# DanecLacey/basic_iterative_solvers

Measured on AMD Instinct MI355X. Metric: CG iterations/sec + SpMV GFLOP/s (% HBM roofline), HPCG 256^3 at 1/2/4/8 GPUs, higher is better.
Workload: dtype f64

## Files before the change

### basic_iterative_solvers_amd/__init__.py

```python
import ctypes as C
import os

import numpy as np

PKG = os.path.dirname(os.path.abspath(__file__))
LIB_PATH = os.path.join(PKG, "lib", "libbis_hip.so")

PC = dict(none=0, j=1, gs=2, bgs=3, sgs=4, **{"2st": 5, "s2st": 6, "ilu0": 7, "ilu0it": 8, "fsai": 9, "mg": 10, "bj": 11})

_lib = None


class BisError(RuntimeError):
    pass


def load_library():
    global _lib
    if _lib is None:
        if not os.path.exists(LIB_PATH):
            raise BisError(
                f"{LIB_PATH} is missing: build it with "
                "`python -m basic_iterative_solvers_amd.build` (hipcc, gfx950)")
        _lib = C.CDLL(LIB_PATH)
# ... 688 lines not shown
                raise BisError("Context.bjacobi: give block_size or block_ptr")
            p = BJParams(int(block_size), None, 0, int(bool(symmetrize)))
        ctx.check(ctx.lib.bis_bj_create(ctx.h, A.h, C.byref(p), C.byref(self.h)))
        self.n_blocks, self.max_block, self.value_count = self.info()
        self.operand = Mat(ctx, C.c_void_p(ctx.lib.bis_bj_operand(self.h)))

    def info(self):
        nb, mb, vc = C.c_int64(), C.c_int(), C.c_int64()
        self.ctx.lib.bis_bj_info(self.h, C.byref(nb), C.byref(mb), C.byref(vc))
        return nb.value, mb.value, vc.value

    def blocks(self):
        vals = np.zeros(self.value_count, dtype=np.float64)
        offs = np.zeros(self.n_blocks + 1, dtype=np.int64)
        self.ctx.check(self.ctx.lib.bis_bj_blocks(self.ctx.h, self.h, vals.ctypes, offs.ctypes))
        return vals, offs

    def apply(self, out, inp):
        self.ctx.check(self.ctx.lib.bis_bj_apply(self.ctx.h, self.h, C.c_void_p(out.ptr), C.c_void_p(inp.ptr)))

    def mapply(self, out, inp, k):
        self.ctx.check(self.ctx.lib.bis_bj_mapply(self.ctx.h, self.h, C.c_void_p(out.ptr), C.c_void_p(inp.ptr), C.c_int(int(k))))

    def free(self):
        if self.h:
            self.ctx.lib.bis_bj_destroy(self.ctx.h, self.h)
            self.h = C.c_void_p()


def _handle_pc(pc, Ls):
    if isinstance(pc, MG):
        return "mg", pc.operand
    if isinstance(pc, BJ):
        return "bj", pc.operand
    return pc, Ls


class _Solver:

    _sym = None

    def _fn(self, what):
        return getattr(self.ctx.lib, f"bis_{self._sym}_{what}")

    def set_preconditioner(self, pc, Ls=None, Us=None, A_D=None, A_D_inv=None, L_D=None, U_D=None, outer=1, inner=0):
        def p(v):
            return C.c_void_p(v.ptr) if v is not None else C.c_void_p()
        pc, Ls = _handle_pc(pc, Ls)
        self._keep_pc = (Ls, Us, A_D, A_D_inv, L_D, U_D)
        self.ctx.check(self._fn("set_preconditioner")(
            self.ctx.h, self.h, C.c_int(PC[pc] if isinstance(pc, str) else pc),
            Ls.h if Ls is not None else C.c_void_p(), Us.h if Us is not None else C.c_void_p(),
            p(A_D), p(A_D_inv), p(L_D), p(U_D), C.c_int(outer), C.c_int(inner)))

    def iterate(self, n):
        self.ctx.check(self._fn("iterate")(self.ctx.h, self.h, C.c_int(int(n))))

    def free(self):
        if self.h:
            self._fn("destroy")(self.ctx.h, self.h)
            self.h = C.c_void_p()


class CG(_Solver):
    _sym = "cg"

    def __init__(self, ctx, A, b, x, A_D=None):
        self.ctx = ctx
        self.h = C.c_void_p()
        ctx.check(ctx.lib.bis_cg_create(ctx.h, A.h, C.c_void_p(A_D.ptr) if A_D else C.c_void_p(),
                                        C.c_void_p(b.ptr), C.c_void_p(x.ptr), C.byref(self.h)))

    def init(self, tol):
        r0 = C.c_double()
        self.ctx.check(self.ctx.lib.bis_cg_init(self.ctx.h, self.h, C.c_double(tol), C.byref(r0)))
        return r0.value

    def status(self, hist_cap=4096):
        iters, conv = C.c_int(), C.c_int()
        hist = np.zeros(hist_cap)
        self.ctx.check(self.ctx.lib.bis_cg_status(self.ctx.h, self.h, C.byref(iters), C.byref(conv),
                                                  hist.ctypes, C.c_int(hist_cap)))
        return iters.value, bool(conv.value), hist[:min(iters.value + 1, hist_cap)].copy()


class MCG(_Solver):

    _sym = "mcg"

    def __init__(self, ctx, A, B, X, k, A_D=None):
        self.ctx, self.k = ctx, int(k)
        self.h = C.c_void_p()
        self._keep = (A, B, X, A_D)
        ctx.check(ctx.lib.bis_mcg_create(ctx.h, A.h, C.c_void_p(A_D.ptr) if A_D else C.c_void_p(),
                                         C.c_void_p(B.ptr), C.c_void_p(X.ptr), C.c_int(self.k), C.byref(self.h)))

    def init(self, tol):
        r0 = np.zeros(self.k)
        self.ctx.check(self.ctx.lib.bis_mcg_init(self.ctx.h, self.h, C.c_double(tol), r0.ctypes))
        return r0

    def status(self, j, hist_cap=4096):
        iters, conv = C.c_int(), C.c_int()
        hist = np.zeros(hist_cap)
        self.ctx.check(self.ctx.lib.bis_mcg_status(self.ctx.h, self.h, C.c_int(int(j)), C.byref(iters), C.byref(conv),
                                                   hist.ctypes, C.c_int(hist_cap)))
        return iters.value, bool(conv.value), hist[:min(iters.value + 1, hist_cap)].copy()


class MBiCGSTAB(_Solver):

    _sym = "mbicgstab"

    def __init__(self, ctx, A, B, X, k):
        self.ctx, self.k = ctx, int(k)
        self.h = C.c_void_p()
        self._keep = (A, B, X)
        ctx.check(ctx.lib.bis_mbicgstab_create(ctx.h, A.h, C.c_void_p(B.ptr), C.c_void_p(X.ptr), C.c_int(self.k), C.byref(self.h)))

    def init(self, tol):
        r0 = np.zeros(self.k)
        self.ctx.check(self.ctx.lib.bis_mbicgstab_init(self.ctx.h, self.h, C.c_double(tol), r0.ctypes))
        return r0

    def status(self, j, hist_cap=4096):
        iters, conv = C.c_int(), C.c_int()
        hist = np.zeros(hist_cap)
        self.ctx.check(self.ctx.lib.bis_mbicgstab_status(self.ctx.h, self.h, C.c_int(int(j)), C.byref(iters), C.byref(conv),
                                                         hist.ctypes, C.c_int(hist_cap)))
        return iters.value, bool(conv.value), hist[:min(iters.value + 1, hist_cap)].copy()


class MGMRES(_Solver):

    _sym = "mgmres"

    def __init__(self, ctx, A, B, X, k, restart=10):
        self.ctx, self.k, self.restart = ctx, int(k), int(restart)
        self.h = C.c_void_p()
        self._keep = (A, B, X)
        ctx.check(ctx.lib.bis_mgmres_create(ctx.h, A.h, C.c_void_p(B.ptr), C.c_void_p(X.ptr), C.c_int(self.k),
                                            C.c_int(self.restart), C.byref(self.h)))

    def init(self, tol):
        r0 = np.zeros(self.k)
        self.ctx.check(self.ctx.lib.bis_mgmres_init(self.ctx.h, self.h, C.c_double(tol), r0.ctypes))
        return r0

    def status(self, j, hist_cap=4096):
        iters, conv, n_hist = C.c_int(), C.c_int(), C.c_int()
        hist = np.zeros(hist_cap)
        self.ctx.check(self.ctx.lib.bis_mgmres_status(self.ctx.h, self.h, C.c_int(int(j)), C.byref(iters), C.byref(conv),
                                                      C.byref(n_hist), hist.ctypes, C.c_int(hist_cap)))
        return iters.value, bool(conv.value), hist[:min(n_hist.value, hist_cap)].copy()

    def solution(self, out):
        self.ctx.check(self.ctx.lib.bis_mgmres_solution(self.ctx.h, self.h, C.c_void_p(out.ptr)))


class FGMRES(_Solver):

    _sym = "fgmres"

    def __init__(self, ctx, A, b, x, restart=10):
        self.ctx, self.restart = ctx, int(restart)
        self.h = C.c_void_p()
# ... 380 lines not shown
```

### basic_iterative_solvers_amd/csrc/bis_blas1.hip

```cpp
#include "bis_internal.hpp"

#include <algorithm>
#include <cstdlib>

namespace {

constexpr int kEwThreads = 256;

inline int ew_grid(int64_t n_items) {
    int64_t g = (n_items + kEwThreads - 1) / kEwThreads;
    if (g < 1) g = 1;
    if (g > kMaxDotBlocks) g = kMaxDotBlocks;
    return (int)g;
}
inline int ew_grid_wide(int64_t n_items) {
    int64_t g = (n_items + kEwThreads - 1) / kEwThreads;
    if (g < 1) g = 1;
    if (g > kMaxEwBlocks) g = kMaxEwBlocks;
    return (int)g;
}

typedef double ew_v2d_t __attribute__((ext_vector_type(2)));
__device__ __forceinline__ double2 ld_stream(const double2 *p) {
    const ew_v2d_t v = __builtin_nontemporal_load(reinterpret_cast<const ew_v2d_t *>(p));
// ... 127 lines not shown
    int64_t i = (int64_t)blockIdx.x * kEwThreads + threadIdx.x;
    double acc0 = 0.0, acc1 = 0.0;
    if (VEC) {
        const int64_t n2 = n >> 1;
        double2 *w2 = reinterpret_cast<double2 *>(w);
        const double2 *u2 = reinterpret_cast<const double2 *>(u);
        const double2 *v2 = reinterpret_cast<const double2 *>(v);
        for (; i < n2; i += stride) {
            double2 wv = ld_stream(w2 + i);
            const double2 uv = ld_stream(u2 + i);
            wv.x = ew_apply<OP_SUB>(wv.x, uv.x, s);
            wv.y = ew_apply<OP_SUB>(wv.y, uv.y, s);
            w2[i] = wv;
            const double2 vv = v ? ld_stream(v2 + i) : wv;
            acc0 = fma(wv.x, vv.x, acc0);
            acc1 = fma(wv.y, vv.y, acc1);
        }
        if ((n & 1) && blockIdx.x == 0 && threadIdx.x == 0) {
            const double t = ew_apply<OP_SUB>(w[n - 1], u[n - 1], s);
            w[n - 1] = t;
            acc0 = fma(t, v ? v[n - 1] : t, acc0);
        }
    } else {
        for (; i < n; i += stride) {
            const double t = ew_apply<OP_SUB>(w[i], u[i], s);
            w[i] = t;
            acc0 = fma(t, v ? v[i] : t, acc0);
        }
    }
    const double r = block_sum<kEwThreads>(acc0 + acc1, lds);
    if (threadIdx.x == 0) partials[blockIdx.x] = r;
}

__global__ __launch_bounds__(256) void reduce_finish_kernel(const double *partials,
                                                            int n_partials, size_t stride,
                                                            double *result) {
    __shared__ double lds[4];
    const double *p = partials + (size_t)blockIdx.x * stride;
    double acc = 0.0;
    for (int i = threadIdx.x; i < n_partials; i += 256) acc += p[i];
    const double s = block_sum<256>(acc, lds);
    if (threadIdx.x == 0) result[blockIdx.x] = s;
}

enum { SC_DIV, SC_RATIO_PRODUCT, SC_SQRT_INV };
__global__ void scalar_kernel(int op, double *out, double *out2, const double *a, const double *b, const double *c,
                              const double *d) {
    if (op == SC_DIV) *out = *a / *b;
    else if (op == SC_RATIO_PRODUCT) *out = (*a / *b) * (*c / *d);
    else { const double nrm = sqrt(*a); *out = nrm; *out2 = 1.0 / nrm; }
}

}

bis_status bis_reduce_finish(bis_ctx *ctx, int n_partials, int n_values, size_t stride,
                             double *result_dev) {
    hipLaunchKernelGGL(reduce_finish_kernel, dim3(n_values), dim3(256), 0, ctx->stream,
                       ctx->partials, n_partials, stride, result_dev);
    BIS_HIP_CHECK(ctx, hipGetLastError());
    return BIS_OK;
}

bis_status bis_ensure_partials(bis_ctx *ctx, size_t n) {
    if (n <= ctx->partials_cap) return BIS_OK;
    BIS_HIP_CHECK(ctx, hipStreamSynchronize(ctx->stream));
    if (ctx->partials) BIS_HIP_CHECK(ctx, hipFree(ctx->partials));
    ctx->partials = nullptr;
    ctx->partials_cap = 0;
    BIS_HIP_CHECK(ctx, hipMalloc(&ctx->partials, sizeof(double) * n));
    ctx->partials_cap = n;
    return BIS_OK;
}

bis_status bis_fault_check(bis_ctx *ctx) {
    volatile unsigned *f = ctx->fault_host;
    if (!f || *f == 0) return BIS_OK;
    *f = 0;
    ctx->err = "a triangular sweep lost a hand-off: a row waited for a result that was never published "
               "(a workgroup of the persistent grid could not become resident, or the dependency data is corrupt); "
               "the vectors written since the last blocking call are invalid";
    return BIS_ERR_SYNC;
}

#define BIS_OPTIONS_ENV(X) X(spmv_variant) X(spmv_window) X(spmv_chunk) X(spmv_chunk_fused) X(spmv_xcd_remap) X(trsv_grid) X(ilu0_wgs) X(trsv_wave_wgs) X(trsv_trial) X(trsv_one_xcd) X(trsv_host_analysis) X(ilu0_wave) X(spmv_packed) X(spmv_packed32) X(spmv_valdict) X(spmv_sellwin) X(device_share) X(spmv_sellwin_rows) X(spmv_sellwin_joint) X(spmv_sellwin_pairs) X(spmv_sellwin_masks) X(spmv_colslab) X(spmv_win8) X(spmv_win8_rows) X(spmv_win8_depth) X(spmv_win8_sets) X(spmv_win8_implicit) X(spmv_win8_tune) X(spmv_win4) X(grid_autodetect) X(tune_placement) X(force_rp64) X(trsv_tiled) X(trsv_chain) X(trsv_tile_rows) X(trsv_tile_wgs) X(trsv_tile_edge) X(trsv_tile_backoff)
#define BIS_OPTIONS_API(Y) Y(trsv_batch) Y(trsv_wave) Y(ilu0_persistent) Y(trsv_by_pos) Y(spmv_lds_pad) Y(trsv_chain_idle) Y(trsv_chain_pause) Y(trsv_chain_pairs) Y(trsv_chain_prefix) Y(trsv_tile_exp) Y(cg_nt_x) Y(spmv_sellwin_nt) Y(dist_host_plan) Y(trsv_inject_loss) Y(trsv_inject_oom) Y(trsm_form) Y(spgemm_row_cap) Y(spgemm_batch)

namespace {
std::string &opts_env_seen() { static std::string s; return s; }
std::string upper_env(const char *name) {
    std::string e = "BIS_";
    for (const char *c = name; *c; ++c) e += (char)((*c >= 'a' && *c <= 'z') ? *c - 32 : *c);
    return e;
}
}

bis_options &bis_opts() {
    static bis_options o = [] {
        bis_options v;
#define X(name) { const std::string en = upper_env(#name); if (const char *e = getenv(en.c_str())) { v.name = atoi(e); \
                  std::string &seen = opts_env_seen(); if (!seen.empty()) seen += ' '; seen += en + "=" + e; } }
        BIS_OPTIONS_ENV(X)
#undef X
        return v;
    }();
    return o;
}

extern "C" {

bis_status bis_set_option(const char *name, int value) {
    if (!name) return BIS_ERR_INVALID;
    bis_options &o = bis_opts();
#define X(opt) if (!strcmp(name, #opt)) { o.opt = value; return BIS_OK; }
    BIS_OPTIONS_ENV(X)
    BIS_OPTIONS_API(X)
#undef X
    return BIS_ERR_INVALID;
}

int bis_options_describe(char *buf, int cap) {
    const bis_options &o = bis_opts();
    std::string s = "{";
    bool first = true;
#define X(opt) if (o.opt != -1) { if (!first) s += ", "; first = false; s += std::string("\"") + #opt + "\": " + std::to_string(o.opt); }
    BIS_OPTIONS_ENV(X)
    BIS_OPTIONS_API(X)
#undef X
    if (!first) s += ", ";
    s += "\"env\": \"";
    for (char c : opts_env_seen()) if (c != '"' && c != '\\' && (unsigned char)c >= 32) s += c;
    s += "\"}";
    if (buf && cap > 0) { const int n = std::min((int)s.size(), cap - 1); memcpy(buf, s.data(), (size_t)n); buf[n] = 0; }
    return (int)s.size();
}

int bis_abi_version(void) { return 1; }

bis_status bis_ctx_create(int device, void *stream, bis_ctx **out) {
    if (!out) return BIS_ERR_INVALID;
    *out = nullptr;
    int count = 0;
    if (hipGetDeviceCount(&count) != hipSuccess || count <= 0) return BIS_ERR_NO_DEVICE;
    if (device < 0 || device >= count) return BIS_ERR_NO_DEVICE;
    if (hipSetDevice(device) != hipSuccess) return BIS_ERR_NO_DEVICE;
    hipDeviceProp_t prop;
    if (hipGetDeviceProperties(&prop, device) != hipSuccess) return BIS_ERR_NO_DEVICE;
    bis_ctx *ctx = new bis_ctx;
    ctx->device = device;
    ctx->n_cus = prop.multiProcessorCount;
    ctx->arch = prop.gcnArchName;
    ctx->hbm_bytes = (int64_t)prop.totalGlobalMem;
    if (ctx->arch.rfind("gfx950", 0) != 0) {
        fprintf(stderr, "bis_hip: device %d is %s, this library is built for gfx950 only\n",
                device, ctx->arch.c_str());
        delete ctx;
        return BIS_ERR_NO_DEVICE;
    }
    if (stream) {
        ctx->stream = (hipStream_t)stream;
    } else {
        if (hipStreamCreateWithFlags(&ctx->stream, hipStreamNonBlocking) != hipSuccess) {
            delete ctx;
            return BIS_ERR_HIP;
        }
        ctx->own_stream = true;
    }
    ctx->partials_cap = std::max((size_t)kMaxReduceBlocks * 4, (size_t)kMaxDotBlocks * 2);
// ... 327 lines not shown
```

### basic_iterative_solvers_amd/csrc/bis_cg.hip

```cpp
#include "bis_solver.hpp"

#include <algorithm>
#include <cfloat>
#include <cmath>

struct bis_dist;
bis_status bis_dist_spmv_launch(bis_ctx *ctx, bis_dist *d, double *x_ext, double *y, const double *w,
                                int *n_partials);
size_t bis_dist_partials_need(const bis_dist *d);
int64_t bis_dist_n_local(const bis_dist *d);
int64_t bis_dist_n_ext(const bis_dist *d);
bis_status bis_dist_allreduce(bis_ctx *ctx, bis_dist *d, double *buf_dev, int count);

struct bis_cg : bis_solver_core {
    bis_dist *dist = nullptr;
    const bis_mat *A = nullptr;
    const double *A_D = nullptr;
    const double *b = nullptr;
    double *x = nullptr;
    int64_t n = 0;
    double *p = nullptr, *r = nullptr, *z = nullptr, *tmp = nullptr;
    double *sc = nullptr;
    double *pap_stage = nullptr;
};

namespace {

enum { S_RZ = 0, S_PAP, S_RZ_NEW, S_RR, S_ALPHA, S_BETA, S_STOP, S_COUNT = 8 };
constexpr int kT = kSolverT;


__device__ __forceinline__ void cg_book(double rz_new, double rr, double *sc, int *flags, double *hist, int hist_cap) {
    const double rz_old = sc[S_RZ];
    sc[S_BETA] = rz_new / rz_old;
    sc[S_RZ] = rz_new;
    sc[S_RR] = rr;
    const double norm = sqrt(rr);
    const int it = flags[0] + 1;
    flags[0] = it;
    if (it < hist_cap) hist[it] = norm;
    const bool conv = fabs(norm) < sc[S_STOP];
    const bool diverged = fabs(norm) > DBL_MAX || norm != norm;
    if (conv || diverged) { flags[1] = 1; flags[2] = conv ? 1 : 0; flags[3] = it; }
}

constexpr int kPapBlocks = 256;
__global__ __launch_bounds__(256) void cg_finish_pap_kernel(const double *__restrict__ partials, int n_partials,
                                                            double *stage, double *sc, const int *flags,
                                                            unsigned *counter) {
    __shared__ double lds[4];
    __shared__ bool last;
    if (flags[1]) return;
    const int per = (n_partials + kPapBlocks - 1) / kPapBlocks;
    const int lo = blockIdx.x * per, hi = min(lo + per, n_partials);
    double acc = 0.0;
    for (int i = lo + (int)threadIdx.x; i < hi; i += 256) acc += partials[i];
    const double s = block_sum<256>(acc, lds);
    if (threadIdx.x == 0) {
        publish(stage + blockIdx.x, s);
        last = arrive_last(counter, kPapBlocks);
    }
    __syncthreads();
    if (!last) return;
    const double t = block_sum<256>(threadIdx.x < kPapBlocks ? fetch(stage + threadIdx.x) : 0.0, lds);
    if (threadIdx.x == 0) sc[S_PAP] = t;
}

typedef double cg_v2d_t __attribute__((ext_vector_type(2)));
template <bool JACOBI, bool DIST>
__global__ __launch_bounds__(kT) void cg_update_kernel(int64_t n, double *sc, int *flags,
                                                       const double *__restrict__ tmp,
                                                       const double *__restrict__ D,
                                                       double *__restrict__ r,
                                                       double *__restrict__ z,
                                                       double *partials, size_t stride, unsigned *counter,
                                                       double *hist, int hist_cap, int nt_tmp, int nt_r) {
    __shared__ double lds[kT / 64];
    __shared__ bool last;
    if (flags[1]) return;
    const double alpha = sc[S_RZ] / sc[S_PAP];
    const int64_t n2 = n >> 1, gs = (int64_t)gridDim.x * kT;
    double rz = 0.0, rr = 0.0;
    const double2 *t2 = reinterpret_cast<const double2 *>(tmp);
    const double2 *D2 = reinterpret_cast<const double2 *>(D);
    double2 *r2 = reinterpret_cast<double2 *>(r);
    double2 *z2 = reinterpret_cast<double2 *>(z);
    for (int64_t i = (int64_t)blockIdx.x * kT + threadIdx.x; i < n2; i += gs) {
        double2 tv;
        if (nt_tmp) {
            const cg_v2d_t v = __builtin_nontemporal_load(reinterpret_cast<const cg_v2d_t *>(t2 + i));
            tv = make_double2(v.x, v.y);
        } else tv = t2[i];
        double2 rv, zv;
        if (nt_r) {
            const cg_v2d_t v = __builtin_nontemporal_load(reinterpret_cast<const cg_v2d_t *>(r2 + i));
            rv = make_double2(v.x, v.y);
        } else rv = r2[i];
        rv.x = fma(-alpha, tv.x, rv.x);
        rv.y = fma(-alpha, tv.y, rv.y);
        r2[i] = rv;
        if (JACOBI) {
            const double2 dv = D2[i];
            zv.x = rv.x / (1.0 * dv.x);
            zv.y = rv.y / (1.0 * dv.y);
            z2[i] = zv;
        } else {
// ... 65 lines not shown
        } else xv = x2[i];
        xv.x = fma(alpha, pv.x, xv.x);
        xv.y = fma(alpha, pv.y, xv.y);
        pv.x = fma(beta, pv.x, zv.x);
        pv.y = fma(beta, pv.y, zv.y);
        if (NT) { cg_v2d_t v; v.x = xv.x; v.y = xv.y; __builtin_nontemporal_store(v, reinterpret_cast<cg_v2d_t *>(x2 + i)); }
        else x2[i] = xv;
        p2[i] = pv;
    }
    if ((n & 1) && blockIdx.x == 0 && threadIdx.x == 0) {
        x[n - 1] = fma(alpha, p[n - 1], x[n - 1]);
        p[n - 1] = fma(beta, p[n - 1], z[n - 1]);
    }
}

}

extern "C" {

static bis_status cg_create_common(bis_ctx *ctx, bis_dist *dist, const bis_mat *A, const double *A_D,
                                   const double *b, double *x, bis_cg **out) {
    bis_cg *cg = new bis_cg;
    cg->dist = dist;
    cg->A = A;
    cg->A_D = A_D;
    cg->b = b;
    cg->x = x;
    cg->n = dist ? bis_dist_n_local(dist) : A->n_rows;
    const int64_t n_ext = dist ? bis_dist_n_ext(dist) : cg->n;
    bis_status st = bis_vec_alloc(ctx, n_ext, &cg->p);
    if (st == BIS_OK) st = bis_vec_alloc(ctx, cg->n, &cg->r);
    if (st == BIS_OK && A_D) st = bis_vec_alloc(ctx, cg->n, &cg->z);
    if (st == BIS_OK) st = bis_vec_alloc(ctx, cg->n, &cg->tmp);
    if (st == BIS_OK) st = bis_vec_alloc(ctx, S_COUNT, &cg->sc);
    if (st == BIS_OK) st = bis_vec_alloc(ctx, kPapBlocks, &cg->pap_stage);
    if (st == BIS_OK) st = bis_solver_core_alloc(ctx, cg, 4, 1, 1, 4 + kArriveSubs);
    if (st != BIS_OK) { bis_cg_destroy(ctx, cg); return st; }
    cg->pc.tmp = cg->tmp;
    if (!A_D) cg->z = cg->r;
    *out = cg;
    return BIS_OK;
}

bis_status bis_cg_create(bis_ctx *ctx, const bis_mat *A, const double *A_D, const double *b,
                         double *x, bis_cg **out) {
    BIS_CTX_OK(ctx);
    BIS_REQUIRE(ctx, A && b && x && out, "bis_cg_create: bad arguments");
    BIS_REQUIRE(ctx, A->n_rows == A->n_cols, "bis_cg_create: square matrix required");
    return cg_create_common(ctx, nullptr, A, A_D, b, x, out);
}

bis_status bis_dist_cg_create(bis_ctx *ctx, bis_dist *d, const double *A_D, const double *b,
                              double *x, bis_cg **out) {
    BIS_CTX_OK(ctx);
    BIS_REQUIRE(ctx, d && b && x && out, "bis_dist_cg_create: bad arguments");
    return cg_create_common(ctx, d, nullptr, A_D, b, x, out);
}

bis_status bis_cg_set_preconditioner(bis_ctx *ctx, bis_cg *cg, int precond_type, const bis_mat *L_strict, const bis_mat *U_strict,
                                     const double *A_D, const double *A_D_inv, const double *L_D, const double *U_D,
                                     int outer_iters, int inner_iters) {
    BIS_CTX_OK(ctx);
    if (!cg) return bis_pc_no_handle(ctx, "bis_cg", 0, precond_type);
    return bis_pc_bind(ctx, &cg->pc, {"bis_cg", cg->n, cg->n, 0, bis_solver_live(*cg), cg->dist ? 2 : 1},
                       {precond_type, L_strict, U_strict, A_D, A_D_inv, L_D, U_D, outer_iters, inner_iters},
                       {{&cg->z, cg->n, cg->z == cg->r}});
}

bis_status bis_cg_destroy(bis_ctx *ctx, bis_cg *cg) {
    BIS_CTX_OK(ctx);
    if (!cg) return BIS_OK;
    hipStreamSynchronize(ctx->stream);
    hipFree(cg->p);
    hipFree(cg->r);
    if (cg->z != cg->r) hipFree(cg->z);
    hipFree(cg->tmp);
    hipFree(cg->sc);
    hipFree(cg->pap_stage);
    bis_solver_core_free(cg);
    delete cg;
    return BIS_OK;
}

bis_status bis_cg_init(bis_ctx *ctx, bis_cg *cg, double tol, double *r0_norm_host) {
    BIS_CTX_OK(ctx);
    BIS_REQUIRE(ctx, cg, "bis_cg_init: null handle");
    const int64_t n = cg->n;
    bis_status st;
    double rz = 0.0, rr = 0.0;
    if (cg->dist) {
        st = bis_copy_vector(ctx, cg->p, cg->x, n);
        if (st == BIS_OK) st = bis_dist_spmv_launch(ctx, cg->dist, cg->p, cg->tmp, nullptr, nullptr);
        if (st == BIS_OK) st = bis_subtract_vectors(ctx, cg->r, cg->b, cg->tmp, n, 1.0);
    } else {
        st = bis_compute_residual(ctx, cg->A, cg->x, cg->b, cg->r, cg->tmp);
    }
    if (st == BIS_OK && cg->pc.set) st = bis_pc_apply(ctx, cg->pc, n, 0, cg->z, cg->r);
    else if (st == BIS_OK && cg->A_D) st = bis_elemwise_div_vectors(ctx, cg->z, cg->r, cg->A_D, n, 1.0);
    if (st == BIS_OK) st = bis_copy_vector(ctx, cg->p, cg->z, n);
    if (cg->dist) {
        if (st == BIS_OK) st = bis_dist_dot(ctx, cg->dist, cg->r, cg->z, ctx->scalars_dev + 8, &rz);
        if (st == BIS_OK) st = bis_dist_dot(ctx, cg->dist, cg->r, cg->r, ctx->scalars_dev + 8, &rr);
    } else {
        if (st == BIS_OK) st = bis_dot(ctx, cg->r, cg->z, n, &rz);
        if (st == BIS_OK) st = bis_dot(ctx, cg->r, cg->r, n, &rr);
    }
    if (st != BIS_OK) return st;
    const double norm0 = sqrt(rr);
    double sc[S_COUNT] = {0};
    sc[S_RZ] = rz;
    sc[S_RR] = rr;
    sc[S_STOP] = tol * norm0;
    int flags[4] = {0, 0, 0, 0};
    BIS_HIP_CHECK(ctx, hipMemcpyAsync(cg->sc, sc, sizeof sc, hipMemcpyHostToDevice, ctx->stream));
    BIS_HIP_CHECK(ctx, hipMemcpyAsync(cg->flags, flags, sizeof flags, hipMemcpyHostToDevice, ctx->stream));
    BIS_HIP_CHECK(ctx, hipMemcpyAsync(cg->hist, &norm0, sizeof(double), hipMemcpyHostToDevice, ctx->stream));
    BIS_HIP_CHECK(ctx, hipStreamSynchronize(ctx->stream));
    cg->enqueued = 0;
    cg->initialised = true;
    if (r0_norm_host) *r0_norm_host = norm0;
    return BIS_OK;
}

static bis_status cg_enqueue_iteration(bis_ctx *ctx, bis_cg *cg, int g, int it) {
    const int64_t n = cg->n;
    int n_part = 0;
    bis_status st;
    if (cg->dist) st = bis_dist_spmv_launch(ctx, cg->dist, cg->p, cg->tmp, cg->p, &n_part);
    else st = bis_spmv_launch(ctx, cg->A, cg->p, cg->tmp, cg->p, &n_part);
    if (st != BIS_OK) return st;
    hipLaunchKernelGGL(cg_finish_pap_kernel, dim3(kPapBlocks), dim3(256), 0, ctx->stream,
                       ctx->partials, n_part, cg->pap_stage, cg->sc, cg->flags, cg->counters);
    if (cg->dist) {
        st = bis_dist_allreduce(ctx, cg->dist, cg->sc + S_PAP, 1);
        if (st != BIS_OK) return st;
    }
#define BIS_CG_UPDATE(J, D)                                                                                  \
    hipLaunchKernelGGL((cg_update_kernel<J, D>), dim3(g), dim3(kT), 0, ctx->stream, n, cg->sc, cg->flags,    \
                       cg->tmp, cg->A_D, cg->r, cg->z, ctx->partials, (size_t)kMaxReduceBlocks,              \
                       cg->counters + 1, cg->hist, cg->hist_cap, bis_opts().cg_nt_x != 0 && bis_opts().cg_nt_x != 2, bis_opts().cg_nt_x == 3)
    if (cg->pc.set) BIS_CG_UPDATE(false, true);
    else if (cg->dist) { if (cg->A_D) BIS_CG_UPDATE(true, true); else BIS_CG_UPDATE(false, true); }
    else { if (cg->A_D) BIS_CG_UPDATE(true, false); else BIS_CG_UPDATE(false, false); }
#undef BIS_CG_UPDATE
    if (cg->pc.set) {
        st = bis_pc_apply(ctx, cg->pc, n, 0, cg->z, cg->r);
        if (st == BIS_OK) st = bis_dot_dev(ctx, cg->r, cg->z, n, cg->sc + S_RZ_NEW);
        if (st != BIS_OK) return st;
        if (!cg->dist)
            hipLaunchKernelGGL(cg_book_kernel, dim3(1), dim3(64), 0, ctx->stream, cg->sc, cg->flags, cg->hist, cg->hist_cap);
    }
    if (cg->dist) {
        st = bis_dist_allreduce(ctx, cg->dist, cg->sc + S_RZ_NEW, 2);
        if (st != BIS_OK) return st;
        hipLaunchKernelGGL(cg_book_kernel, dim3(1), dim3(64), 0, ctx->stream, cg->sc, cg->flags, cg->hist, cg->hist_cap);
    }
    if (bis_opts().cg_nt_x == 3) hipLaunchKernelGGL((cg_p_update_kernel<true, true>), dim3(g), dim3(kT), 0, ctx->stream, n, cg->sc, cg->flags, it, cg->z, cg->x, cg->p);
    else if (bis_opts().cg_nt_x != 0) hipLaunchKernelGGL(cg_p_update_kernel<true>, dim3(g), dim3(kT), 0, ctx->stream, n, cg->sc, cg->flags, it, cg->z, cg->x, cg->p);
    else hipLaunchKernelGGL(cg_p_update_kernel<false>, dim3(g), dim3(kT), 0, ctx->stream, n, cg->sc, cg->flags, it, cg->z, cg->x, cg->p);
    return BIS_OK;
}

bis_status bis_cg_iterate(bis_ctx *ctx, bis_cg *cg, int n_iters) {
    BIS_CTX_OK(ctx);
    BIS_REQUIRE(ctx, cg && n_iters >= 0 && cg->enqueued + n_iters < kMaxIters,
                "bis_cg_iterate: bad arguments");
    const int64_t n = cg->n;
    if (n == 0) return BIS_OK;
    const int g = bis_pair_grid(n, kMaxReduceBlocks);
    const size_t need = std::max((size_t)2 * kMaxReduceBlocks,
                                 cg->dist ? bis_dist_partials_need(cg->dist) : bis_spmv_partials_bound(cg->A));
    bis_status st = bis_ensure_partials(ctx, need);
    if (st != BIS_OK) return st;
    bis_stop_guard stop_guard(ctx, cg->flags);
    for (int done = 0; done < n_iters; ++done) {
        st = cg_enqueue_iteration(ctx, cg, g, cg->enqueued + done + 1);
        if (st != BIS_OK) { cg->enqueued += done; return st; }
    }
    BIS_HIP_CHECK(ctx, hipGetLastError());
    cg->enqueued += n_iters;
    return BIS_OK;
}

bis_status bis_cg_status(bis_ctx *ctx, bis_cg *cg, int *iters, int *converged, double *hist_host,
                         int hist_cap) {
    BIS_CTX_OK(ctx);
    BIS_REQUIRE(ctx, cg, "bis_cg_status: null handle");
    int flags[4] = {0, 0, 0, 0};
    if (bis_status st = bis_solver_read_flags(ctx, *cg, 0, 4, flags)) return st;
    if (iters) *iters = flags[0];
    if (converged) *converged = flags[2];
    if (hist_host && hist_cap > 0) return bis_solver_copy_hist(ctx, *cg, 0, std::min(flags[0] + 1, hist_cap), hist_host);
    return BIS_OK;
}

}
```

### basic_iterative_solvers_amd/csrc/bis_internal.hpp

```cpp
#pragma once

#include <hip/hip_runtime.h>

#include <cstdint>
#include <cstdio>
#include <cstring>
#include <map>
#include <string>
#include <vector>

#include "bis_hip.h"

struct bis_trsv_plan;
struct bis_trsv_tiled;
struct bis_trsv_chain;
struct bis_trsm_plan;
struct bis_trsv_side {
    bis_trsv_plan *level = nullptr;
    bis_trsv_tiled *tiled = nullptr;
    bis_trsv_chain *chain = nullptr;
    bis_trsm_plan *multi = nullptr;
    bool tiled_tried = false, chain_tried = false;
    const char *kernel = "";
    const char *kernel_m = "";
};

struct bis_named_kernel {
    int type = 0;
    const bis_mat *A = nullptr;
    double *B = nullptr, *C = nullptr;
    int64_t size_B = 0, size_C = 0;
    const double *D = nullptr;
    bool upper = false;
};

struct bis_ctx {
    int device = 0;
    hipStream_t stream = nullptr;
    bool own_stream = false;
    int n_cus = 0;
    std::string arch;
    int64_t hbm_bytes = 0;
    std::string err;

    double *partials = nullptr;
    size_t partials_cap = 0;
    double *scalars_dev = nullptr;
    double *scalars_host = nullptr;
    unsigned *counters = nullptr;
    unsigned *fault_host = nullptr, *fault_dev = nullptr;

    std::map<std::string, bis_named_kernel> kernels;

    const int *spmv_stop = nullptr;

    bool profile = false;
    std::vector<std::pair<hipEvent_t, hipEvent_t>> prof_events;
    size_t prof_used = 0;
    std::vector<std::pair<hipEvent_t, hipEvent_t>> prof_sweep_events;
    size_t prof_sweep_used = 0;
};

struct bis_options;
bis_options &bis_opts();
struct bis_options {
    int spmv_variant = -1;
    int spmv_window = -1;
    int spmv_chunk = -1;
    int spmv_chunk_fused = -1;
    int spmv_xcd_remap = -1;
    int trsv_grid = -1;
    int ilu0_wave = -1;
    int ilu0_wgs = -1;
    int ilu0_persistent = -1;
    int trsv_host_analysis = -1;
    int trsv_wave = -1;
    int trsv_wave_wgs = -1;
    int trsv_trial = -1;
    int trsv_batch = -1;
    int trsv_by_pos = -1;
    int trsv_one_xcd = -1;
    int tune_placement = -1;
    int spmv_packed32 = -1;
    int spmv_lds_pad = -1;
    int spmv_packed = -1;
    int spmv_valdict = -1;
    int dist_host_plan = -1;
    int grid_autodetect = -1;
    int trsv_chain = -1;
    int trsv_chain_idle = -1;
    int trsv_chain_pause = -1;
    int trsv_chain_prefix = -1;
    int trsv_chain_pairs = -1;
    int trsv_tiled = -1;
    int trsv_tile_rows = -1;
    int trsv_tile_wgs = -1;
    int trsv_tile_backoff = -1;
    int spmv_sellwin_nt = -1;
    int cg_nt_x = -1;
    int trsv_tile_exp = -1;
    int trsv_tile_edge = -1;
    int force_rp64 = -1;
    int spmv_sellwin = -1;
    int spmv_sellwin_rows = -1;
    int spmv_sellwin_pairs = -1;
    int spmv_sellwin_joint = -1;
    int spmv_colslab = -1;
    int spmv_win8 = -1;
    int spmv_win8_rows = -1;
    int spmv_win8_depth = -1;
    int spmv_win8_sets = -1;
    int spmv_win8_implicit = -1;
    int spmv_win8_tune = -1;
    int spmv_win4 = -1;
    int spmv_sellwin_masks = -1;
    int device_share = -1;
    int trsm_form = -1;
    int spgemm_row_cap = -1;
    int spgemm_batch = -1;
    int trsv_inject_oom = -1;
    int trsv_inject_loss = -1;
};
inline bool bis_want_rp64(int64_t nnz) { return nnz >= (int64_t)INT32_MAX - 8 || bis_opts().force_rp64 > 0; }

constexpr int kMaxReduceBlocks = 2048;
constexpr int kMaxDotBlocks = 8192;
constexpr int kMaxEwBlocks = 16384;
constexpr int kMaxIters = 1 << 20;
constexpr int kWinMaxTiles = 128;
constexpr int kWinTile = 16;
constexpr int kWinTileLog = 4;
constexpr int kSwRows = 256;
constexpr int kSwMaxR = 4;

struct bis_mat {
    int64_t n_rows = 0, n_cols = 0, nnz = 0;
    bool rp64 = false;
    bool view = false;
    void *row_ptr = nullptr;
    int32_t *col = nullptr;
    double *val = nullptr;
    int32_t *blk_row = nullptr;
    int64_t *blk_nnz = nullptr;
    int n_blocks = 0;
    int64_t view_row0 = 0;
    struct bis_xwin *xw = nullptr;
    struct { struct bis_colpack *p = nullptr; int state = 0; } pk[2];
    struct { struct bis_valdict *p = nullptr; int state = 0; } vd;
    struct bis_sellwin *sw = nullptr;
    int sw_state = 0;
    struct { struct bis_win8 *p = nullptr; int state = 0; } w8[2];
    struct { std::vector<bis_mat *> *slabs = nullptr; int state = 0; double trial_ms[2] = {0.0, 0.0}; } cs;
    bool f32_exact = false;
    int32_t *blkf_row = nullptr;
    int64_t *blkf_nnz = nullptr;
    int n_blocks_f = 0;
    int chunk_f = 0;
    int chunk_nnz = 0;
    int max_row_nnz = 0;
    int64_t max_block_nnz = 0;
    int64_t grid[4] = {0, 0, 0, 0};
    bis_trsv_side trsv[2];
    const char *spmv_kernel[2] = {"", ""};
    const char *ilu0_kernel = "";
    const char *itrsv_kernel = "";
    const char *spmm_kernel = "";
    const char *iluk_kernel = "";
    const char *spgemm_kernel = "";
    const char *fsai_kernel = "";
    struct bis_mg *mg = nullptr;
    struct bis_bj *bj = nullptr;
};

#define BIS_HIP_CHECK(ctx, call)                                               \
    do {                                                                       \
        hipError_t e_ = (call);                                                \
        if (e_ != hipSuccess) {                                                \
            (ctx)->err = std::string(#call) + ": " + hipGetErrorString(e_);    \
            return BIS_ERR_HIP;                                                \
        }                                                                      \
    } while (0)

// ... 196 lines not shown
```

### basic_iterative_solvers_amd/csrc/bis_solver.hpp

```cpp
#pragma once

#include "bis_pc.hpp"

#include <algorithm>

struct bis_solver_core {
    int *flags = nullptr;
    double *hist = nullptr;
    int hist_cap = 0;
    int enqueued = 0;
    bool initialised = false;
    unsigned *counters = nullptr;
    bis_pc_binding pc;
};

bis_status bis_solver_core_alloc(bis_ctx *ctx, bis_solver_core *core, size_t n_flags, int hist_cols, int n_counter_sets,
                                 unsigned set_words);
void bis_solver_core_free(bis_solver_core *core);
inline bool bis_solver_live(const bis_solver_core &core) { return core.initialised || core.enqueued != 0; }
bis_status bis_solver_read_flags(bis_ctx *ctx, const bis_solver_core &core, size_t offset, int count, int *out);
bis_status bis_solver_copy_hist(bis_ctx *ctx, const bis_solver_core &core, int j, int cnt, double *hist_host);

struct bis_stop_guard {
    bis_ctx *ctx;
    bis_stop_guard(bis_ctx *c, const int *flags) : ctx(c) { c->spmv_stop = flags; }
    ~bis_stop_guard() { ctx->spmv_stop = nullptr; }
    bis_stop_guard(const bis_stop_guard &) = delete;
    bis_stop_guard &operator=(const bis_stop_guard &) = delete;
};

constexpr int kSolverT = 256;
inline int bis_pair_grid(int64_t n, int cap) {
    const int64_t g = ((n >> 1) + kSolverT - 1) / kSolverT;
    return (int)std::min<int64_t>(std::max<int64_t>(g, 1), cap);
}

constexpr unsigned kCounterSubBase = 4;
constexpr unsigned bis_counter_set_words(unsigned max_blocks) {
    return kCounterSubBase + (max_blocks + kArriveGroup - 1) / kArriveGroup;
}
__device__ __forceinline__ bool arrive_last_set(unsigned *set, unsigned block, unsigned n_blocks) {
    return arrive_last2(set, set + kCounterSubBase, block, n_blocks);
}

template <int NV>
__device__ __forceinline__ bool reduce_last(const double (&acc)[NV], double *lds , double *partials,
                                            unsigned *counter, double (&total)[NV]) {
    __shared__ bool last;
#pragma unroll
    for (int v = 0; v < NV; ++v) {
        const double sum = block_sum<kSolverT>(acc[v], lds + v * (kSolverT / 64));
        if (threadIdx.x == 0) publish(partials + (size_t)v * gridDim.x + blockIdx.x, sum);
    }
    if (threadIdx.x == 0) last = arrive_last_set(counter, blockIdx.x, gridDim.x);
    __syncthreads();
    if (!last) return false;
#pragma unroll
    for (int v = 0; v < NV; ++v) {
        double a = 0.0;
        for (int i = threadIdx.x; i < (int)gridDim.x; i += kSolverT) a += fetch(partials + (size_t)v * gridDim.x + i);
        total[v] = block_sum<kSolverT>(a, lds + v * (kSolverT / 64));
    }
    return true;
}
```

### include/bis_hip.h

```cpp
#ifndef BIS_HIP_H
#define BIS_HIP_H

#include <stddef.h>
#include <stdint.h>

#ifdef __cplusplus
extern "C" {
#endif

#define BIS_API __attribute__((visibility("default")))

typedef int bis_status;
enum {
    BIS_OK = 0,
    BIS_ERR_NO_DEVICE = 1,
    BIS_ERR_INVALID = 2,
    BIS_ERR_HIP = 3,
    BIS_ERR_ZERO_DIAG = 4,
    BIS_ERR_NO_DIAG = 5,
    BIS_ERR_UNSUPPORTED = 6,
    BIS_ERR_COMM = 7,
    BIS_ERR_SYNC = 8
};

// ... 231 lines not shown
                             double scalar, int64_t n);
BIS_API bis_status bis_init_vector(bis_ctx *ctx, double *v, double val,
                                   int64_t n);
BIS_API bis_status bis_copy_vector(bis_ctx *ctx, double *out, const double *in,
                                   int64_t n);
BIS_API bis_status bis_normalize_x(bis_ctx *ctx, double *x_new,
                                   const double *x_old, const double *D,
                                   const double *b, int64_t n);
BIS_API bis_status bis_multi_axpy(bis_ctx *ctx, const double *V, int64_t ldv,
                                  const double *y_host, int n_vec, double *out,
                                  int64_t n);
BIS_API bis_status bis_two_stage_gauss_seidel(bis_ctx *ctx,
                                              const bis_mat *strict,
                                              double *tmp, double *work,
                                              const double *D_inv,
                                              const double *input,
                                              double *output, int64_t n,
                                              int inner_iters);
BIS_API bis_status bis_itrsv(bis_ctx *ctx, const bis_mat *T_strict, const double *D_inv,
                             const double *b, double *x, double *work, int n_sweeps);
BIS_API const char *bis_itrsv_kernel(const bis_mat *T_strict);
BIS_API bis_status bis_apply_preconditioner(
    bis_ctx *ctx, int precond_type, int64_t n, const bis_mat *L_strict,
    const bis_mat *U_strict, const double *A_D, const double *A_D_inv,
    const double *L_D, const double *U_D, double *output, double *input,
    double *tmp, double *work, int outer_iters, int inner_iters);

BIS_API bis_status bis_sptrsm(bis_ctx *ctx, const bis_mat *L_strict, double *X, const double *D, const double *B, int n_rhs);
BIS_API bis_status bis_bsptrsm(bis_ctx *ctx, const bis_mat *U_strict, double *X, const double *D, const double *B, int n_rhs);
BIS_API const char *bis_mat_sweepm_kernel(const bis_mat *T, int backward);
BIS_API bis_status bis_mvec_div_diag(bis_ctx *ctx, double *R, const double *A, const double *D, int64_t n, int n_rhs);
BIS_API bis_status bis_mvec_mul_diag(bis_ctx *ctx, double *R, const double *A, const double *D, int64_t n, int n_rhs);
BIS_API bis_status bis_mitrsv(bis_ctx *ctx, const bis_mat *T_strict, const double *D_inv, const double *B, double *X,
                              double *WORK, int n_sweeps, int n_rhs);
BIS_API bis_status bis_mapply_preconditioner(
    bis_ctx *ctx, int precond_type, int64_t n, int n_rhs, const bis_mat *L_strict,
    const bis_mat *U_strict, const double *A_D, const double *A_D_inv,
    const double *L_D, const double *U_D, double *OUT, double *IN,
    double *TMP, double *WORK, int outer_iters, int inner_iters);

enum { BIS_KERNEL_SPMV = 0, BIS_KERNEL_SPTRSV = 1 };
BIS_API bis_status bis_register_kernel(bis_ctx *ctx, const char *name, int type);
BIS_API bis_status bis_kernel_register_A(bis_ctx *ctx, const char *name,
                                         const bis_mat *A);
BIS_API bis_status bis_kernel_register_B(bis_ctx *ctx, const char *name,
                                         int64_t size, double *vec);
BIS_API bis_status bis_kernel_register_C(bis_ctx *ctx, const char *name,
                                         int64_t size, double *vec);
BIS_API bis_status bis_kernel_register_D(bis_ctx *ctx, const char *name,
                                         const double *diag);
BIS_API bis_status bis_kernel_set_mat_upper_triang(bis_ctx *ctx,
                                                   const char *name, int flag);
BIS_API bis_status bis_kernel_run(bis_ctx *ctx, const char *name,
                                  int64_t A_offset, int64_t B_offset,
                                  int64_t C_offset);
BIS_API bis_status bis_kernel_swap_operands(bis_ctx *ctx, const char *name);

enum { BIS_STAT_JACOBI = 0, BIS_STAT_GS = 1, BIS_STAT_SGS = 2 };
typedef struct bis_stat bis_stat;
BIS_API bis_status bis_stat_create(bis_ctx *ctx, int kind, const bis_mat *A,
                                   const bis_mat *L_strict, const bis_mat *U_strict,
                                   const double *D, const double *b, double *x,
                                   bis_stat **out);
BIS_API bis_status bis_stat_init(bis_ctx *ctx, bis_stat *s, double tol,
                                 double *r0_norm_host);
BIS_API bis_status bis_stat_iterate(bis_ctx *ctx, bis_stat *s, int n_iters);
BIS_API bis_status bis_stat_status(bis_ctx *ctx, bis_stat *s, int *iters,
                                   int *converged, double *hist_host, int hist_cap);
BIS_API bis_status bis_stat_solution(bis_ctx *ctx, bis_stat *s, double *x_out);
BIS_API bis_status bis_stat_destroy(bis_ctx *ctx, bis_stat *s);

typedef struct bis_cg bis_cg;
BIS_API bis_status bis_cg_create(bis_ctx *ctx, const bis_mat *A,
                                 const double *A_D, const double *b, double *x,
                                 bis_cg **out);
BIS_API bis_status bis_cg_destroy(bis_ctx *ctx, bis_cg *cg);
BIS_API bis_status bis_cg_set_preconditioner(bis_ctx *ctx, bis_cg *cg, int precond_type,
                                             const bis_mat *L_strict, const bis_mat *U_strict,
                                             const double *A_D, const double *A_D_inv,
                                             const double *L_D, const double *U_D,
                                             int outer_iters, int inner_iters);
BIS_API bis_status bis_cg_init(bis_ctx *ctx, bis_cg *cg, double tol,
                               double *r0_norm_host);
BIS_API bis_status bis_cg_iterate(bis_ctx *ctx, bis_cg *cg, int n_iters);
BIS_API bis_status bis_cg_status(bis_ctx *ctx, bis_cg *cg, int *iters,
                                 int *converged, double *hist_host,
                                 int hist_cap);

typedef struct bis_mcg bis_mcg;
BIS_API bis_status bis_mcg_create(bis_ctx *ctx, const bis_mat *A, const double *A_D, const double *B, double *X,
                                  int n_rhs, bis_mcg **out);
BIS_API bis_status bis_mcg_set_preconditioner(bis_ctx *ctx, bis_mcg *m, int precond_type,
                                              const bis_mat *L_strict, const bis_mat *U_strict,
                                              const double *A_D, const double *A_D_inv,
                                              const double *L_D, const double *U_D,
                                              int outer_iters, int inner_iters);
BIS_API bis_status bis_mcg_init(bis_ctx *ctx, bis_mcg *m, double tol, double *r0_norms_host);
BIS_API bis_status bis_mcg_iterate(bis_ctx *ctx, bis_mcg *m, int n_iters);
BIS_API bis_status bis_mcg_status(bis_ctx *ctx, bis_mcg *m, int j, int *iters, int *converged, double *hist_host,
                                  int hist_cap);
BIS_API bis_status bis_mcg_destroy(bis_ctx *ctx, bis_mcg *m);

typedef struct bis_mbicgstab bis_mbicgstab;
BIS_API bis_status bis_mbicgstab_create(bis_ctx *ctx, const bis_mat *A, const double *B, double *X, int n_rhs,
                                        bis_mbicgstab **out);
BIS_API bis_status bis_mbicgstab_set_preconditioner(bis_ctx *ctx, bis_mbicgstab *m, int precond_type,
                                                    const bis_mat *L_strict, const bis_mat *U_strict,
                                                    const double *A_D, const double *A_D_inv,
                                                    const double *L_D, const double *U_D,
                                                    int outer_iters, int inner_iters);
BIS_API bis_status bis_mbicgstab_init(bis_ctx *ctx, bis_mbicgstab *m, double tol, double *r0_norms_host);
BIS_API bis_status bis_mbicgstab_iterate(bis_ctx *ctx, bis_mbicgstab *m, int n_iters);
BIS_API bis_status bis_mbicgstab_status(bis_ctx *ctx, bis_mbicgstab *m, int j, int *iters, int *converged,
                                        double *hist_host, int hist_cap);
BIS_API bis_status bis_mbicgstab_destroy(bis_ctx *ctx, bis_mbicgstab *m);

typedef struct bis_mgmres bis_mgmres;
BIS_API bis_status bis_mgmres_create(bis_ctx *ctx, const bis_mat *A, const double *B, double *X, int n_rhs,
                                     int restart_len, bis_mgmres **out);
BIS_API bis_status bis_mgmres_set_preconditioner(bis_ctx *ctx, bis_mgmres *m, int precond_type,
                                                 const bis_mat *L_strict, const bis_mat *U_strict,
                                                 const double *A_D, const double *A_D_inv,
                                                 const double *L_D, const double *U_D,
                                                 int outer_iters, int inner_iters);
BIS_API bis_status bis_mgmres_init(bis_ctx *ctx, bis_mgmres *m, double tol, double *r0_norms_host);
BIS_API bis_status bis_mgmres_iterate(bis_ctx *ctx, bis_mgmres *m, int n_iters);
BIS_API bis_status bis_mgmres_solution(bis_ctx *ctx, bis_mgmres *m, double *X_out);
BIS_API bis_status bis_mgmres_status(bis_ctx *ctx, bis_mgmres *m, int j, int *iters, int *converged, int *n_hist,
                                     double *hist_host, int hist_cap);
BIS_API bis_status bis_mgmres_destroy(bis_ctx *ctx, bis_mgmres *m);

typedef struct bis_fgmres bis_fgmres;
BIS_API bis_status bis_fgmres_create(bis_ctx *ctx, const bis_mat *A, const double *b, double *x, int restart_len,
                                     bis_fgmres **out);
BIS_API bis_status bis_fgmres_set_preconditioner(bis_ctx *ctx, bis_fgmres *s, int precond_type,
                                                 const bis_mat *L_strict, const bis_mat *U_strict,
                                                 const double *A_D, const double *A_D_inv,
                                                 const double *L_D, const double *U_D,
                                                 int outer_iters, int inner_iters);
BIS_API bis_status bis_fgmres_init(bis_ctx *ctx, bis_fgmres *s, double tol, double *r0_norm_host);
BIS_API bis_status bis_fgmres_iterate(bis_ctx *ctx, bis_fgmres *s, int n_iters);
BIS_API bis_status bis_fgmres_solution(bis_ctx *ctx, bis_fgmres *s, double *x_out);
BIS_API bis_status bis_fgmres_status(bis_ctx *ctx, bis_fgmres *s, int *iters, int *converged, int *n_hist,
                                     double *hist_host, int hist_cap);
BIS_API bis_status bis_fgmres_destroy(bis_ctx *ctx, bis_fgmres *s);

typedef struct bis_minres bis_minres;
BIS_API bis_status bis_minres_create(bis_ctx *ctx, const bis_mat *A, const double *b, double *x, bis_minres **out);
BIS_API bis_status bis_minres_set_preconditioner(bis_ctx *ctx, bis_minres *s, int precond_type,
                                                 const bis_mat *L_strict, const bis_mat *U_strict,
                                                 const double *A_D, const double *A_D_inv,
                                                 const double *L_D, const double *U_D,
                                                 int outer_iters, int inner_iters);
BIS_API bis_status bis_minres_init(bis_ctx *ctx, bis_minres *s, double tol, double *r0_norm_host);
BIS_API bis_status bis_minres_iterate(bis_ctx *ctx, bis_minres *s, int n_iters);
BIS_API bis_status bis_minres_status(bis_ctx *ctx, bis_minres *s, int *iters, int *converged, double *hist_host,
                                     int hist_cap);
BIS_API bis_status bis_minres_destroy(bis_ctx *ctx, bis_minres *s);

typedef struct bis_idr bis_idr;
BIS_API bis_status bis_idr_create(bis_ctx *ctx, const bis_mat *A, const double *b, double *x, int s, bis_idr **out);
BIS_API bis_status bis_idr_set_preconditioner(bis_ctx *ctx, bis_idr *h, int precond_type,
                                              const bis_mat *L_strict, const bis_mat *U_strict,
                                              const double *A_D, const double *A_D_inv,
                                              const double *L_D, const double *U_D,
                                              int outer_iters, int inner_iters);
// ... 107 lines not shown
```

Measured before the change: 1221.

## Search CG work-vector allocations for the fastest physical placement at init

On the first CG init, the solver times a few short CG runs and re-allocates the p, r, tmp (and z) vectors up to several times. It keeps the set whose step time is lowest, aiming to escape unlucky physical address placements that cause channel or cache conflicts against the matrix stream. This adds one-time init cost and temporarily holds extra device memory, and it only runs for single-device unpreconditioned CG. The default is -1, so the search runs only when the win8 stream recorded a kept time, with a target slack added.

```diff
diff --git a/basic_iterative_solvers_amd/__init__.py b/basic_iterative_solvers_amd/__init__.py
--- a/basic_iterative_solvers_amd/__init__.py
+++ b/basic_iterative_solvers_amd/__init__.py
@@ -794,6 +794,12 @@
         self.ctx.check(self.ctx.lib.bis_cg_status(self.ctx.h, self.h, C.byref(iters), C.byref(conv),
                                                   hist.ctypes, C.c_int(hist_cap)))
         return iters.value, bool(conv.value), hist[:min(iters.value + 1, hist_cap)].copy()
+
+    def placement(self):
+        t = C.c_int()
+        v = [C.c_double() for _ in range(4)]
+        self.ctx.lib.bis_cg_placement(self.h, C.byref(t), *[C.byref(x) for x in v])
+        return dict(zip(("first_spmv_ms", "kept_spmv_ms", "first_step_ms", "kept_step_ms"), (x.value for x in v)), trials=t.value)
 
 
 class MCG(_Solver):
diff --git a/basic_iterative_solvers_amd/csrc/bis_blas1.hip b/basic_iterative_solvers_amd/csrc/bis_blas1.hip
--- a/basic_iterative_solvers_amd/csrc/bis_blas1.hip
+++ b/basic_iterative_solvers_amd/csrc/bis_blas1.hip
@@ -233,7 +233,7 @@
     return BIS_ERR_SYNC;
 }
 
-#define BIS_OPTIONS_ENV(X) X(spmv_variant) X(spmv_window) X(spmv_chunk) X(spmv_chunk_fused) X(spmv_xcd_remap) X(trsv_grid) X(ilu0_wgs) X(trsv_wave_wgs) X(trsv_trial) X(trsv_one_xcd) X(trsv_host_analysis) X(ilu0_wave) X(spmv_packed) X(spmv_packed32) X(spmv_valdict) X(spmv_sellwin) X(device_share) X(spmv_sellwin_rows) X(spmv_sellwin_joint) X(spmv_sellwin_pairs) X(spmv_sellwin_masks) X(spmv_colslab) X(spmv_win8) X(spmv_win8_rows) X(spmv_win8_depth) X(spmv_win8_sets) X(spmv_win8_implicit) X(spmv_win8_tune) X(spmv_win4) X(grid_autodetect) X(tune_placement) X(force_rp64) X(trsv_tiled) X(trsv_chain) X(trsv_tile_rows) X(trsv_tile_wgs) X(trsv_tile_edge) X(trsv_tile_backoff)
+#define BIS_OPTIONS_ENV(X) X(spmv_variant) X(spmv_window) X(spmv_chunk) X(spmv_chunk_fused) X(spmv_xcd_remap) X(trsv_grid) X(ilu0_wgs) X(trsv_wave_wgs) X(trsv_trial) X(trsv_one_xcd) X(trsv_host_analysis) X(ilu0_wave) X(spmv_packed) X(spmv_packed32) X(spmv_valdict) X(spmv_sellwin) X(device_share) X(spmv_sellwin_rows) X(spmv_sellwin_joint) X(spmv_sellwin_pairs) X(spmv_sellwin_masks) X(spmv_colslab) X(spmv_win8) X(spmv_win8_rows) X(spmv_win8_depth) X(spmv_win8_sets) X(spmv_win8_implicit) X(spmv_win8_tune) X(spmv_win4) X(cg_place) X(grid_autodetect) X(tune_placement) X(force_rp64) X(trsv_tiled) X(trsv_chain) X(trsv_tile_rows) X(trsv_tile_wgs) X(trsv_tile_edge) X(trsv_tile_backoff)
 #define BIS_OPTIONS_API(Y) Y(trsv_batch) Y(trsv_wave) Y(ilu0_persistent) Y(trsv_by_pos) Y(spmv_lds_pad) Y(trsv_chain_idle) Y(trsv_chain_pause) Y(trsv_chain_pairs) Y(trsv_chain_prefix) Y(trsv_tile_exp) Y(cg_nt_x) Y(spmv_sellwin_nt) Y(dist_host_plan) Y(trsv_inject_loss) Y(trsv_inject_oom) Y(trsm_form) Y(spgemm_row_cap) Y(spgemm_batch)
 
 namespace {
diff --git a/basic_iterative_solvers_amd/csrc/bis_cg.hip b/basic_iterative_solvers_amd/csrc/bis_cg.hip
--- a/basic_iterative_solvers_amd/csrc/bis_cg.hip
+++ b/basic_iterative_solvers_amd/csrc/bis_cg.hip
@@ -3,6 +3,8 @@
 #include <algorithm>
 #include <cfloat>
 #include <cmath>
+#include <cstdio>
+#include <cstdlib>
 
 struct bis_dist;
 bis_status bis_dist_spmv_launch(bis_ctx *ctx, bis_dist *d, double *x_ext, double *y, const double *w,
@@ -22,6 +24,8 @@
     double *p = nullptr, *r = nullptr, *z = nullptr, *tmp = nullptr;
     double *sc = nullptr;
     double *pap_stage = nullptr;
+    bool placed = false;
+    bis_place_report place;
 };
 
 namespace {
@@ -253,9 +257,7 @@
     return BIS_OK;
 }
 
-bis_status bis_cg_init(bis_ctx *ctx, bis_cg *cg, double tol, double *r0_norm_host) {
-    BIS_CTX_OK(ctx);
-    BIS_REQUIRE(ctx, cg, "bis_cg_init: null handle");
+static bis_status cg_init_state(bis_ctx *ctx, bis_cg *cg, double tol, double *r0_norm_host) {
     const int64_t n = cg->n;
     bis_status st;
     double rz = 0.0, rr = 0.0;
@@ -293,6 +295,89 @@
     return BIS_OK;
 }
 
+static bis_status cg_enqueue(bis_ctx *ctx, bis_cg *cg, int n_iters);
+
+static bis_status cg_place_trial(bis_ctx *ctx, bis_cg *cg, double *x_save, bis_private_prof &prof, hipEvent_t e0, hipEvent_t e1,
+                                 double *spmv_ms, double *step_ms) {
+    const int n_timed = 5;
+    bis_status st = bis_copy_vector(ctx, x_save, cg->x, cg->n);
+    if (st != BIS_OK) return st;
+    st = cg_init_state(ctx, cg, 0.0, nullptr);
+    if (st == BIS_OK) st = cg_enqueue(ctx, cg, 2);
+    if (st == BIS_OK) {
+        hipEventRecord(e0, ctx->stream);
+        prof.begin();
+        st = cg_enqueue(ctx, cg, n_timed);
+        hipEventRecord(e1, ctx->stream);
+        float f = 0.f;
+        if (hipEventSynchronize(e1) != hipSuccess || !prof.read(spmv_ms) || hipEventElapsedTime(&f, e0, e1) != hipSuccess) {
+            (void)hipGetLastError();
+            if (st == BIS_OK) { ctx->err = "bis_cg_init: the placement trial could not be timed"; st = BIS_ERR_HIP; }
+        }
+        *step_ms = f / (double)n_timed;
+    }
+    const bis_status back = bis_copy_vector(ctx, cg->x, x_save, cg->n);
+    return st != BIS_OK ? st : back;
+}
+
+static bis_status cg_place(bis_ctx *ctx, bis_cg *cg) {
+    const int opt = bis_opts().cg_place;
+    if (cg->dist || cg->pc.set || opt == 0 || cg->n == 0) return BIS_OK;
+    int form = 0;
+    if (bis_status st = bis_mat_spmv_stream_info(ctx, cg->A, nullptr, nullptr, nullptr, &form)) return st;
+    double kept_ms = 0.0;
+    if (form == 6 || form == 8) bis_mat_win8_tuning(cg->A, nullptr, nullptr, &kept_ms);
+    if (opt < 0 && kept_ms <= 0.0) return BIS_OK;
+    double *x_save = nullptr;
+    hipEvent_t e0 = nullptr, e1 = nullptr;
+    if (hipMalloc(reinterpret_cast<void **>(&x_save), sizeof(double) * (size_t)cg->n) != hipSuccess || hipEventCreate(&e0) != hipSuccess ||
+        hipEventCreate(&e1) != hipSuccess) {
+        (void)hipGetLastError();
+        hipFree(x_save);
+        if (e0) hipEventDestroy(e0);
+        return BIS_OK;
+    }
+    std::vector<bis_place_vec> vecs = {{&cg->p, cg->n}, {&cg->r, cg->n}, {&cg->tmp, cg->n}};
+    if (cg->A_D) vecs.push_back({&cg->z, cg->n});
+    auto follow = [&]() { cg->pc.tmp = cg->tmp; if (!cg->A_D) cg->z = cg->r; };
+    bis_status st;
+    {
+        bis_private_prof prof(ctx);
+        st = bis_place_search(ctx, vecs, opt > 0 ? opt : 6, kept_ms > 0.0 ? kept_ms + 0.03 : 0.0,
+                              [&](double *spmv_ms, double *step_ms) { follow(); return cg_place_trial(ctx, cg, x_save, prof, e0, e1, spmv_ms, step_ms); },
+                              &cg->place);
+    }
+    follow();
+    hipStreamSynchronize(ctx->stream);
+    hipFree(x_save);
+    hipEventDestroy(e0);
+    hipEventDestroy(e1);
+    if (st == BIS_OK && getenv("BIS_CG_PLACE_STATS"))
+        fprintf(stderr, "cg placement: %d re-allocation(s) of %d vectors of %lld rows tried, in-loop SpMV %.4f ms on the first set, %.4f ms on the one kept (stream's kept time %.4f ms); step %.4f ms on the first set, %.4f ms on the one kept\n",
+                cg->place.trials, (int)vecs.size(), (long long)cg->n, cg->place.first_spmv_ms, cg->place.kept_spmv_ms, kept_ms, cg->place.first_step_ms, cg->place.kept_step_ms);
+    return st;
+}
+
+bis_status bis_cg_init(bis_ctx *ctx, bis_cg *cg, double tol, double *r0_norm_host) {
+    BIS_CTX_OK(ctx);
+    BIS_REQUIRE(ctx, cg, "bis_cg_init: null handle");
+    if (!cg->placed) {
+        cg->placed = true;
+        if (bis_status st = cg_place(ctx, cg)) return st;
+    }
+    return cg_init_state(ctx, cg, tol, r0_norm_host);
+}
+
+void bis_cg_placement(const bis_cg *cg, int *trials, double *first_spmv_ms, double *kept_spmv_ms, double *first_step_ms, double *kept_step_ms) {
+    const bis_place_report none;
+    const bis_place_report &p = cg ? cg->place : none;
+    if (trials) *trials = p.trials;
+    if (first_spmv_ms) *first_spmv_ms = p.first_spmv_ms;
+    if (kept_spmv_ms) *kept_spmv_ms = p.kept_spmv_ms;
+    if (first_step_ms) *first_step_ms = p.first_step_ms;
+    if (kept_step_ms) *kept_step_ms = p.kept_step_ms;
+}
+
 static bis_status cg_enqueue_iteration(bis_ctx *ctx, bis_cg *cg, int g, int it) {
     const int64_t n = cg->n;
     int n_part = 0;
@@ -336,6 +421,10 @@
     BIS_CTX_OK(ctx);
     BIS_REQUIRE(ctx, cg && n_iters >= 0 && cg->enqueued + n_iters < kMaxIters,
                 "bis_cg_iterate: bad arguments");
+    return cg_enqueue(ctx, cg, n_iters);
+}
+
+static bis_status cg_enqueue(bis_ctx *ctx, bis_cg *cg, int n_iters) {
     const int64_t n = cg->n;
     if (n == 0) return BIS_OK;
     const int g = bis_pair_grid(n, kMaxReduceBlocks);
diff --git a/basic_iterative_solvers_amd/csrc/bis_internal.hpp b/basic_iterative_solvers_amd/csrc/bis_internal.hpp
--- a/basic_iterative_solvers_amd/csrc/bis_internal.hpp
+++ b/basic_iterative_solvers_amd/csrc/bis_internal.hpp
@@ -98,6 +98,7 @@
     int trsv_tile_backoff = -1;
     int spmv_sellwin_nt = -1;
     int cg_nt_x = -1;
+    int cg_place = -1;
     int trsv_tile_exp = -1;
     int trsv_tile_edge = -1;
     int force_rp64 = -1;
diff --git a/basic_iterative_solvers_amd/csrc/bis_solver.hpp b/basic_iterative_solvers_amd/csrc/bis_solver.hpp
--- a/basic_iterative_solvers_amd/csrc/bis_solver.hpp
+++ b/basic_iterative_solvers_amd/csrc/bis_solver.hpp
@@ -3,6 +3,8 @@
 #include "bis_pc.hpp"
 
 #include <algorithm>
+#include <utility>
+#include <vector>
 
 struct bis_solver_core {
     int *flags = nullptr;
@@ -28,6 +30,86 @@
     bis_stop_guard(const bis_stop_guard &) = delete;
     bis_stop_guard &operator=(const bis_stop_guard &) = delete;
 };
+
+struct bis_place_report {
+    int trials = 0;
+    double first_spmv_ms = 0.0, kept_spmv_ms = 0.0;
+    double first_step_ms = 0.0, kept_step_ms = 0.0;
+};
+struct bis_place_vec { double **slot; int64_t n; };
+
+struct bis_private_prof {
+    bis_ctx *ctx;
+    bool was_on;
+    size_t was_used;
+    std::vector<std::pair<hipEvent_t, hipEvent_t>> callers;
+    explicit bis_private_prof(bis_ctx *c) : ctx(c), was_on(c->profile), was_used(c->prof_used) {
+        callers.swap(c->prof_events);
+        c->prof_used = 0;
+        c->profile = false;
+    }
+    ~bis_private_prof() {
+        for (auto &p : ctx->prof_events) { hipEventDestroy(p.first); hipEventDestroy(p.second); }
+        ctx->prof_events.clear();
+        ctx->prof_events.swap(callers);
+        ctx->prof_used = was_used;
+        ctx->profile = was_on;
+    }
+    void begin() { ctx->prof_used = 0; ctx->profile = true; }
+    bool read(double *ms_per_launch) {
+        ctx->profile = false;
+        if (hipStreamSynchronize(ctx->stream) != hipSuccess) return false;
+        double ms = 0.0;
+        for (size_t i = 0; i < ctx->prof_used; ++i) {
+            float t = 0.f;
+            if (hipEventElapsedTime(&t, ctx->prof_events[i].first, ctx->prof_events[i].second) != hipSuccess) return false;
+            ms += t;
+        }
+        *ms_per_launch = ctx->prof_used ? ms / (double)ctx->prof_used : 0.0;
+        ctx->prof_used = 0;
+        return true;
+    }
+    bis_private_prof(const bis_private_prof &) = delete;
+    bis_private_prof &operator=(const bis_private_prof &) = delete;
+};
+
+template <class Trial>
+bis_status bis_place_search(bis_ctx *ctx, const std::vector<bis_place_vec> &vecs, int k, double target_spmv_ms, Trial &&trial,
+                            bis_place_report *rep) {
+    const size_t nv = vecs.size();
+    size_t bytes = 0;
+    std::vector<double *> best(nv), losers;
+    for (size_t i = 0; i < nv; ++i) { best[i] = *vecs[i].slot; bytes += sizeof(double) * (size_t)std::max<int64_t>(vecs[i].n, 1); }
+    double spmv = 0.0, step = 0.0;
+    bis_status st = trial(&spmv, &step);
+    if (st != BIS_OK) return st;
+    *rep = {0, spmv, spmv, step, step};
+    while (rep->trials < k && !(target_spmv_ms > 0.0 && spmv <= target_spmv_ms)) {
+        size_t free_b = 0, total_b = 0;
+        if (hipMemGetInfo(&free_b, &total_b) != hipSuccess || free_b < bytes + ((size_t)8 << 30)) break;
+        std::vector<double *> cand(nv, nullptr);
+        bool ok = true;
+        for (size_t i = 0; i < nv && ok; ++i)
+            ok = hipMalloc(reinterpret_cast<void **>(&cand[i]), sizeof(double) * (size_t)std::max<int64_t>(vecs[i].n, 1)) == hipSuccess;
+        if (!ok) { (void)hipGetLastError(); for (double *p : cand) hipFree(p); break; }
+        for (size_t i = 0; i < nv; ++i) *vecs[i].slot = cand[i];
+        st = trial(&spmv, &step);
+        ++rep->trials;
+        if (st == BIS_OK && step < rep->kept_step_ms) {
+            losers.insert(losers.end(), best.begin(), best.end());
+            best = cand;
+            rep->kept_spmv_ms = spmv;
+            rep->kept_step_ms = step;
+        } else {
+            losers.insert(losers.end(), cand.begin(), cand.end());
+        }
+        if (st != BIS_OK) break;
+    }
+    for (size_t i = 0; i < nv; ++i) *vecs[i].slot = best[i];
+    hipStreamSynchronize(ctx->stream);
+    for (double *p : losers) hipFree(p);
+    return st;
+}
 
 constexpr int kSolverT = 256;
 inline int bis_pair_grid(int64_t n, int cap) {
diff --git a/include/bis_hip.h b/include/bis_hip.h
--- a/include/bis_hip.h
+++ b/include/bis_hip.h
@@ -337,6 +337,8 @@
                                              int outer_iters, int inner_iters);
 BIS_API bis_status bis_cg_init(bis_ctx *ctx, bis_cg *cg, double tol,
                                double *r0_norm_host);
+BIS_API void bis_cg_placement(const bis_cg *cg, int *trials, double *first_spmv_ms, double *kept_spmv_ms,
+                              double *first_step_ms, double *kept_step_ms);
 BIS_API bis_status bis_cg_iterate(bis_ctx *ctx, bis_cg *cg, int n_iters);
 BIS_API bis_status bis_cg_status(bis_ctx *ctx, bis_cg *cg, int *iters,
                                  int *converged, double *hist_host,
```

Result: slower. 1194 (-2.2%).
